# wuji3/visiondk

Measured on AMD Instinct MI355X. Metric: images/sec fwd+bwd+optimizer step (ViT-B/16, bs=256 per GPU), higher is better.
Workload: dtype fp16; 1 GPU; ViT-B/16 ICT, synthetic ImageNet-1k 224x224, random-init weights (reference re-init), per-GPU batch 256, CE label_smoothing 0.05, SGD 0.006/0.937/5e-4, clip 10, EMA on rank 0; global_batch=256, parallelism=dp1

## Files before the change

### visiondk_amd/csrc/norm_loss.hip

```cpp
#include <hip/hip_runtime.h>
#include "vdk_device.h"
#include "vdk_host.h"

__device__ __forceinline__ unsigned ln_q8_pack4(const u32x2 bf, float s, float lim, int fmt, float& am) {
  float c[4];
#pragma unroll
  for (int e = 0; e < 2; ++e) {
    const float a = bf_lo(bf[e]), b = bf_hi(bf[e]);
    am = fmaxf(am, fmaxf(fabsf(a), fabsf(b)));
    c[2 * e] = fminf(fmaxf(a * s, -lim), lim); c[2 * e + 1] = fminf(fmaxf(b * s, -lim), lim);
  }
  int v = 0;
  if (fmt == 0) { v = __builtin_amdgcn_cvt_pk_fp8_f32(c[0], c[1], v, false); v = __builtin_amdgcn_cvt_pk_fp8_f32(c[2], c[3], v, true); }
  else { v = __builtin_amdgcn_cvt_pk_bf8_f32(c[0], c[1], v, false); v = __builtin_amdgcn_cvt_pk_bf8_f32(c[2], c[3], v, true); }
  return (unsigned)v;
}
__device__ __forceinline__ void ln_q8_publish(float am, float* amax, int lane, float* red4) {
#pragma unroll
  for (int off = 1; off < 64; off <<= 1) am = fmaxf(am, __shfl_xor(am, off));
  if (lane == 0) red4[threadIdx.x >> 6] = am;
  __syncthreads();
  if (threadIdx.x == 0 && amax) {
    const float m = fmaxf(fmaxf(red4[0], red4[1]), fmaxf(red4[2], red4[3]));
    if (m > *(volatile float*)amax) atomicMax((unsigned*)amax, __float_as_uint(m));
  }
}
template <bool OUT_BF16 , int MAXJ, bool Q8 = false, int OF = 0>
__global__ __launch_bounds__(256) void ln_fwd_kernel(const float* __restrict__ x, long ldx, int T, int C,
                                                     const float* __restrict__ gamma, const float* __restrict__ beta,
                                                     float eps, void* __restrict__ y, long ldy, float* __restrict__ mean,
                                                     float* __restrict__ rstd, LnQ8 q8 = LnQ8()) {
  const int lane = threadIdx.x & 63;
  __shared__ float q8red[4];
  float q8s = 1.0f, q8lim = 448.0f, q8am = 0.f;
  if (Q8) { q8s = q8.scale ? q8.scale[0] : 1.0f; q8lim = q8.fmt == 0 ? 448.0f : 57344.0f; }
  const int rstride = Q8 ? (int)gridDim.x * 4 : T;
  for (int row = blockIdx.x * 4 + (threadIdx.x >> 6); row < T; row += rstride) {
  const float* xr = x + (long)row * ldx;
  f32x4 v[MAXJ];
#pragma unroll
  for (int j = 0; j < MAXJ; ++j) { const int c = lane * 4 + j * 256; if (c < C) v[j] = *(const f32x4*)(xr + c); }
  float s = 0.f;
#pragma unroll
  for (int j = 0; j < MAXJ; ++j) { const int c = lane * 4 + j * 256; if (c < C) s += (v[j][0] + v[j][1]) + (v[j][2] + v[j][3]); }
  const float mu = wave_sum(s) / (float)C;
  float q = 0.f;
#pragma unroll
  for (int j = 0; j < MAXJ; ++j) {
    const int c = lane * 4 + j * 256;
    if (c < C) {
#pragma unroll
      for (int e = 0; e < 4; ++e) { float d = v[j][e] - mu; q = fmaf(d, d, q); }
    }
  }
  const float rs = 1.0f / sqrtf(wave_sum(q) / (float)C + eps);
  if (lane == 0) { if (mean) mean[row] = mu; if (rstd) rstd[row] = rs; }
#pragma unroll
  for (int j = 0; j < MAXJ; ++j) {
    const int c = lane * 4 + j * 256;
    if (c < C) {
      f32x4 g = *(const f32x4*)(gamma + c), b = *(const f32x4*)(beta + c);
      float o[4];
#pragma unroll
      for (int e = 0; e < 4; ++e) o[e] = (v[j][e] - mu) * rs * g[e] + b[e];
      if (OUT_BF16) {
        const u32x2 ob = {pack_op2<OF>(o[0], o[1]), pack_op2<OF>(o[2], o[3])};
        *(u32x2*)((bf16_t*)y + (long)row * ldy + c) = ob;
        if (Q8) *(unsigned*)(q8.out + (long)row * q8.ld + c) = ln_q8_pack4(ob, q8s, q8lim, q8.fmt, q8am);
      }
      else *(f32x4*)((float*)y + (long)row * ldy + c) = (f32x4){o[0], o[1], o[2], o[3]};
    }
  }
  }
  if (Q8) ln_q8_publish(q8am, q8.amax, lane, q8red);
}

template <bool OUT_BF16, int OF = 0>
__global__ __launch_bounds__(256) void ln_fwd_narrow_kernel(const float* __restrict__ x, long ldx, int T, int C, const float* __restrict__ gamma,
                                                            const float* __restrict__ beta, float eps, void* __restrict__ y, long ldy, float* __restrict__ mean,
                                                            float* __restrict__ rstd) {
  const int row = blockIdx.x * 8 + (threadIdx.x >> 5);
  const int l32 = threadIdx.x & 31, c = l32 * 4;
  const bool on = row < T && c < C;
  f32x4 v = {0.f, 0.f, 0.f, 0.f};
  if (on) v = *(const f32x4*)(x + (long)row * ldx + c);
  float s = on ? (v[0] + v[1]) + (v[2] + v[3]) : 0.f;
#pragma unroll
  for (int o = 16; o >= 1; o >>= 1) s += __shfl_xor(s, o);
  const float mu = s / (float)C;
  float q = 0.f;
  if (on) {
#pragma unroll
    for (int e = 0; e < 4; ++e) { float d = v[e] - mu; q = fmaf(d, d, q); }
  }
#pragma unroll
  for (int o = 16; o >= 1; o >>= 1) q += __shfl_xor(q, o);
  const float rs = 1.0f / sqrtf(q / (float)C + eps);
  if (row < T && l32 == 0) { if (mean) mean[row] = mu; if (rstd) rstd[row] = rs; }
  if (on) {
    f32x4 g = *(const f32x4*)(gamma + c), b = *(const f32x4*)(beta + c);
    float o4[4];
#pragma unroll
    for (int e = 0; e < 4; ++e) o4[e] = (v[e] - mu) * rs * g[e] + b[e];
    if (OUT_BF16) *(u32x2*)((bf16_t*)y + (long)row * ldy + c) = (u32x2){pack_op2<OF>(o4[0], o4[1]), pack_op2<OF>(o4[2], o4[3])};
    else *(f32x4*)((float*)y + (long)row * ldy + c) = (f32x4){o4[0], o4[1], o4[2], o4[3]};
  }
}

template <int MAXJ, bool DY_BF16 , bool OCS, bool Q8 = false, int OF = 0 , int NR = 1,
          bool HALF = false, bool DR16 = false >
__global__ __launch_bounds__(256) void ln_bwd_kernel(const void* __restrict__ dy, long lddy, const float* __restrict__ x,
                                                     long ldx, const float* __restrict__ mean, const float* __restrict__ rstd,
                                                     const float* __restrict__ gamma, const float* __restrict__ dres,
                                                     long lddres, int T, int C, int rows_per_block, float* __restrict__ dx,
                                                     long lddx, bf16_t* __restrict__ dxb, long lddxb,
                                                     float* __restrict__ pgamma, float* __restrict__ pbeta, float* __restrict__ pout, LnQ8 q8 = LnQ8(),
                                                     const float* __restrict__ dy_scale = nullptr ,
                                                     const float* __restrict__ dxb_rs = nullptr , int dxb_rps = 1,
                                                     const bf16_t* __restrict__ dres16 = nullptr) {
  static_assert(!HALF || MAXJ == 1, "HALF: one 128-column slab");
  __shared__ float red[4][MAXJ * 256];
  float q8s = 1.0f, q8lim = 448.0f, q8am = 0.f;
  if (Q8) { q8s = q8.scale ? q8.scale[0] : 1.0f; q8lim = q8.fmt == 0 ? 448.0f : 57344.0f; }
  const int w = threadIdx.x >> 6, lane = threadIdx.x & 63;
  constexpr int HS = HALF ? 2 : 1, RW = NR * HS;
  const int cl = HALF ? (lane & 31) : lane, sub = HALF ? (lane >> 5) : 0;
  const int r0 = blockIdx.x * rows_per_block;
  int r1 = r0 + rows_per_block; if (r1 > T) r1 = T;
  float ag[MAXJ][4], ab[MAXJ][4], ao[OCS ? MAXJ : 1][4];
#pragma unroll
  for (int j = 0; j < MAXJ; ++j)
#pragma unroll
    for (int e = 0; e < 4; ++e) { ag[j][e] = 0.f; ab[j][e] = 0.f; if (OCS) ao[j][e] = 0.f; }
  const float invC = 1.0f / (float)C;
  const float dsc = dy_scale ? dy_scale[0] : 1.0f;
  for (int rb = r0 + w * RW; rb < r1; rb += 4 * RW) {
    float rs[NR], s1[NR], s2[NR];
    float gk[NR][MAXJ][4], xh[NR][MAXJ][4], rv[NR][MAXJ][4];
#pragma unroll
    for (int k = 0; k < NR; ++k) {
      const int row = rb + k * HS + sub;
      const bool ok = row < r1;
      const float mu = ok ? mean[row] : 0.f;
      rs[k] = ok ? rstd[row] : 0.f;
      s1[k] = 0.f; s2[k] = 0.f;
#pragma unroll
      for (int j = 0; j < MAXJ; ++j) {
        const int c = cl * 4 + j * 256;
#pragma unroll
        for (int e = 0; e < 4; ++e) { gk[k][j][e] = 0.f; xh[k][j][e] = 0.f; rv[k][j][e] = 0.f; }
        if (ok && c < C) {
          f32x4 xv = *(const f32x4*)(x + (long)row * ldx + c);
          f32x4 gm = *(const f32x4*)(gamma + c);
          float d[4];
          if (DY_BF16) {
            u32x2 u = *(const u32x2*)((const bf16_t*)dy + (long)row * lddy + c);
            d[0] = op_lo<OF>(u[0]); d[1] = op_hi<OF>(u[0]); d[2] = op_lo<OF>(u[1]); d[3] = op_hi<OF>(u[1]);
          } else {
            f32x4 u = *(const f32x4*)((const float*)dy + (long)row * lddy + c);
            d[0] = u[0]; d[1] = u[1]; d[2] = u[2]; d[3] = u[3];
          }
          if (dy_scale) { d[0] *= dsc; d[1] *= dsc; d[2] *= dsc; d[3] *= dsc; }
          if (DR16) {
            const u32x2 r2 = *(const u32x2*)(dres16 + (long)row * lddres + c);
            rv[k][j][0] = op_lo<OF>(r2[0]); rv[k][j][1] = op_hi<OF>(r2[0]); rv[k][j][2] = op_lo<OF>(r2[1]); rv[k][j][3] = op_hi<OF>(r2[1]);
          } else if (dres) {
            f32x4 r4 = *(const f32x4*)(dres + (long)row * lddres + c);
            rv[k][j][0] = r4[0]; rv[k][j][1] = r4[1]; rv[k][j][2] = r4[2]; rv[k][j][3] = r4[3];
          }
#pragma unroll
          for (int e = 0; e < 4; ++e) {
            float h = (xv[e] - mu) * rs[k];
            float g = d[e] * gm[e];
            xh[k][j][e] = h; gk[k][j][e] = g;
            s1[k] += g; s2[k] = fmaf(g, h, s2[k]);
            ag[j][e] = fmaf(d[e], h, ag[j][e]);
            ab[j][e] += d[e];
          }
        }
      }
    }
#pragma unroll
    for (int k = 0; k < NR; ++k) {
#pragma unroll
      for (int m = HALF ? 16 : 32; m >= 1; m >>= 1) { s1[k] += __shfl_xor(s1[k], m); s2[k] += __shfl_xor(s2[k], m); }
      s1[k] *= invC; s2[k] *= invC;
    }
#pragma unroll
    for (int k = 0; k < NR; ++k) {
      const int row = rb + k * HS + sub;
      const bool ok = row < r1;
#pragma unroll
      for (int j = 0; j < MAXJ; ++j) {
        const int c = cl * 4 + j * 256;
        if (ok && c < C) {
          float o[4];
#pragma unroll
          for (int e = 0; e < 4; ++e) o[e] = rs[k] * (gk[k][j][e] - s1[k] - xh[k][j][e] * s2[k]) + rv[k][j][e];
          if (dx) *(f32x4*)(dx + (long)row * lddx + c) = (f32x4){o[0], o[1], o[2], o[3]};
          if (dxb) {
            if (dxb_rs) { const float f = dxb_rs[row / dxb_rps]; o[0] *= f; o[1] *= f; o[2] *= f; o[3] *= f; }
            const u32x2 ob = {pack_op2<OF>(o[0], o[1]), pack_op2<OF>(o[2], o[3])};
            *(u32x2*)(dxb + (long)row * lddxb + c) = ob;
            if (OCS) { ao[j][0] += op_lo<OF>(ob[0]); ao[j][1] += op_hi<OF>(ob[0]); ao[j][2] += op_lo<OF>(ob[1]); ao[j][3] += op_hi<OF>(ob[1]); }
            if (Q8) *(unsigned*)(q8.out + (long)row * q8.ld + c) = ln_q8_pack4(ob, q8s, q8lim, q8.fmt, q8am);
          }
        }
      }
    }
  }
  if (Q8) ln_q8_publish(q8am, q8.amax, lane, &red[0][0]);
#pragma unroll
  for (int ph = 0; ph < (OCS ? 3 : 2); ++ph) {
    if (ph) __syncthreads();
#pragma unroll
    for (int j = 0; j < MAXJ; ++j)
#pragma unroll
      for (int e = 0; e < 4; ++e) red[w][j * 256 + lane * 4 + e] = ph == 0 ? ag[j][e] : (ph == 1 ? ab[j][e] : ao[OCS ? j : 0][e]);
    __syncthreads();
    for (int c = threadIdx.x; c < C; c += 256) {
      float v = (red[0][c] + red[1][c]) + (red[2][c] + red[3][c]);
      if (HALF) v += (red[0][c + 128] + red[1][c + 128]) + (red[2][c + 128] + red[3][c + 128]);
      if (ph == 0) pgamma[(long)blockIdx.x * 2 * C + c] = v;
      else if (ph == 1) pbeta[(long)blockIdx.x * 2 * C + c] = v;
      else pout[(long)blockIdx.x * C + c] = v;
    }
  }
}

__global__ __launch_bounds__(512) void reduce_rows_f32_kernel(const float* __restrict__ in, long ld, int S, long n,
                                                              float* __restrict__ out, float scale) {
  __shared__ float red[8][64];
  const int cl = threadIdx.x & 63, rg = threadIdx.x >> 6;
  const long c = (long)blockIdx.x * 64 + cl;
  float s0 = 0.f, s1 = 0.f;
  if (c < n) {
    int k = rg;
    for (; k + 8 < S; k += 16) { s0 += in[(long)k * ld + c]; s1 += in[(long)(k + 8) * ld + c]; }
    if (k < S) s0 += in[(long)k * ld + c];
  }
  red[rg][cl] = s0 + s1;
  __syncthreads();
  if (rg == 0 && c < n)
    out[c] = (((red[0][cl] + red[1][cl]) + (red[2][cl] + red[3][cl])) + ((red[4][cl] + red[5][cl]) + (red[6][cl] + red[7][cl]))) * scale;
}

struct ReduceBatch { VdkReduceJob job[8]; int first_block[9]; int n; };
__global__ __launch_bounds__(512) void reduce_rows_batch_kernel(ReduceBatch b) {
  __shared__ float red[8][64];
  int j = 0;
  while (j + 1 < b.n && (int)blockIdx.x >= b.first_block[j + 1]) ++j;
  const VdkReduceJob jb = b.job[j];
  const int cl = threadIdx.x & 63, rg = threadIdx.x >> 6;
  const long c = (long)((int)blockIdx.x - b.first_block[j]) * 64 + cl;
  float s0 = 0.f, s1 = 0.f;
  if (c < jb.n) {
    int k = rg;
    for (; k + 8 < jb.S; k += 16) { s0 += jb.in[(long)k * jb.ld + c]; s1 += jb.in[(long)(k + 8) * jb.ld + c]; }
    if (k < jb.S) s0 += jb.in[(long)k * jb.ld + c];
  }
  red[rg][cl] = s0 + s1;
  __syncthreads();
  if (rg == 0 && c < jb.n)
    jb.out[c] = (((red[0][cl] + red[1][cl]) + (red[2][cl] + red[3][cl])) + ((red[4][cl] + red[5][cl]) + (red[6][cl] + red[7][cl]))) * jb.scale;
}

__global__ __launch_bounds__(512) void reduce_rows_batch_tall_kernel(ReduceBatch b) {
  __shared__ float red[32][17];
  int j = 0;
  while (j + 1 < b.n && (int)blockIdx.x >= b.first_block[j + 1]) ++j;
  const VdkReduceJob jb = b.job[j];
  const int cl = threadIdx.x & 15, rg = threadIdx.x >> 4;
  const long c = (long)((int)blockIdx.x - b.first_block[j]) * 16 + cl;
  float s0 = 0.f, s1 = 0.f, s2 = 0.f, s3 = 0.f;
  if (c < jb.n) {
    int k = rg;
    for (; k + 96 < jb.S; k += 128) {
      s0 += jb.in[(long)k * jb.ld + c]; s1 += jb.in[(long)(k + 32) * jb.ld + c]; s2 += jb.in[(long)(k + 64) * jb.ld + c]; s3 += jb.in[(long)(k + 96) * jb.ld + c];
    }
    for (; k < jb.S; k += 32) s0 += jb.in[(long)k * jb.ld + c];
  }
  red[rg][cl] = (s0 + s1) + (s2 + s3);
  __syncthreads();
  if (rg == 0 && c < jb.n) {
    float t[8];
#pragma unroll
    for (int g = 0; g < 8; ++g) t[g] = (red[4 * g][cl] + red[4 * g + 1][cl]) + (red[4 * g + 2][cl] + red[4 * g + 3][cl]);
    jb.out[c] = (((t[0] + t[1]) + (t[2] + t[3])) + ((t[4] + t[5]) + (t[6] + t[7]))) * jb.scale;
// ... 248 lines not shown
    return vdk_fail(VDK_EINVAL, "vdk_layernorm_fwd: bad argument (C, ldx, ldy % 4 == 0)");
  if (T == 0) return VDK_OK;
  if (C > 4096) return vdk_fail(VDK_EUNSUPPORTED, "vdk_layernorm_fwd: C <= 4096");
  dim3 grid((unsigned)((T + 3) / 4));
#define LNF(BF, MJ) do { if (f16) hipLaunchKernelGGL((ln_fwd_kernel<true, MJ, false, VDK_OPF_F16>), grid, dim3(256), 0, (hipStream_t)stream, x, (long)ldx, (int)T, (int)C, gamma, beta, eps, y, (long)ldy, mean, rstd); \
                          else hipLaunchKernelGGL((ln_fwd_kernel<BF, MJ>), grid, dim3(256), 0, (hipStream_t)stream, x, (long)ldx, (int)T, (int)C, gamma, beta, eps, y, (long)ldy, mean, rstd); } while (0)
  if (y_dtype != VDK_BF16 && y_dtype != VDK_F32 && y_dtype != VDK_F16) return vdk_fail(VDK_EINVAL, "vdk_layernorm_fwd: bad y_dtype");
  const bool bf = y_dtype == VDK_BF16, f16 = y_dtype == VDK_F16;
  if (C <= 128) {
    const dim3 g8((unsigned)((T + 7) / 8));
    if (f16) hipLaunchKernelGGL((ln_fwd_narrow_kernel<true, VDK_OPF_F16>), g8, dim3(256), 0, (hipStream_t)stream, x, (long)ldx, (int)T, (int)C, gamma, beta, eps, y, (long)ldy, mean, rstd);
    else if (bf) hipLaunchKernelGGL((ln_fwd_narrow_kernel<true>), g8, dim3(256), 0, (hipStream_t)stream, x, (long)ldx, (int)T, (int)C, gamma, beta, eps, y, (long)ldy, mean, rstd);
    else hipLaunchKernelGGL((ln_fwd_narrow_kernel<false>), g8, dim3(256), 0, (hipStream_t)stream, x, (long)ldx, (int)T, (int)C, gamma, beta, eps, y, (long)ldy, mean, rstd);
  }
  else if (C <= 256) { if (bf) LNF(true, 1); else LNF(false, 1); }
  else if (C <= 1024) { if (bf) LNF(true, 4); else LNF(false, 4); }
  else { if (bf) LNF(true, 16); else LNF(false, 16); }
#undef LNF
  return vdk_check_launch("vdk_layernorm_fwd");
}

int vdk_layernorm_fwd_q8(const float* x, int64_t ldx, int32_t T, int32_t C, const float* gamma, const float* beta, float eps, void* y, int64_t ldy, float* mean, float* rstd,
                         void* out8, int64_t ldo8, int32_t out_fmt, const float* out_scale, float* out_amax, void* stream) {
  if (!x || !gamma || !beta || !y || !out8 || T < 0 || C <= 0 || (C & 3) || (ldx & 3) || (ldy & 3) || (ldo8 & 3) || (out_fmt != 0 && out_fmt != 1))
    return vdk_fail(VDK_EINVAL, "vdk_layernorm_fwd_q8: bad argument (C, ldx, ldy, ldo8 % 4 == 0)");
  if (C <= 128 || C > 1024) return vdk_fail(VDK_EUNSUPPORTED, "vdk_layernorm_fwd_q8: 128 < C <= 1024");
  if (T == 0) return VDK_OK;
  const LnQ8 q8 = {(unsigned char*)out8, (long)ldo8, out_scale, out_amax, (int)out_fmt};
  unsigned nblk = (unsigned)((T + 3) / 4); if (nblk > 1024) nblk = 1024;
  if (C <= 256)
    hipLaunchKernelGGL((ln_fwd_kernel<true, 1, true>), dim3(nblk), dim3(256), 0, (hipStream_t)stream, x, (long)ldx, (int)T, (int)C, gamma, beta, eps, y, (long)ldy,
                       mean, rstd, q8);
  else
    hipLaunchKernelGGL((ln_fwd_kernel<true, 4, true>), dim3(nblk), dim3(256), 0, (hipStream_t)stream, x, (long)ldx, (int)T, (int)C, gamma, beta, eps, y, (long)ldy,
                       mean, rstd, q8);
  return vdk_check_launch("vdk_layernorm_fwd_q8");
}

int vdk_reduce_rows_f32(const float* in, int64_t ld, int32_t S, int64_t n, float* out, float scale, void* stream) {
  if (!in || !out || S < 0 || n < 0) return vdk_fail(VDK_EINVAL, "vdk_reduce_rows_f32: bad argument");
  if (n == 0) return VDK_OK;
  hipLaunchKernelGGL(reduce_rows_f32_kernel, dim3((unsigned)((n + 63) / 64)), dim3(512), 0, (hipStream_t)stream, in, (long)ld,
                     (int)S, (long)n, out, scale);
  return vdk_check_launch("vdk_reduce_rows_f32");
}

static inline int ln_bwd_blocks(int T, int C) {
  int nb = (T + 15) / 16;
  const int slots = C <= 768 ? 1024 : 768;
  if (nb > slots) nb = slots;
  if (nb < 1) nb = 1;
  const int rpb = (T + nb - 1) / nb;
  nb = (T + rpb - 1) / rpb;
  return nb;
}
int vdk_layernorm_bwd_workspace_bytes(int32_t T, int32_t C, size_t* bytes) {
  if (!bytes || T < 0 || C <= 0) return vdk_fail(VDK_EINVAL, "vdk_layernorm_bwd_workspace_bytes: bad argument");
  *bytes = (size_t)3 * ln_bwd_blocks(T, C) * C * 4;
  return VDK_OK;
}
static int ln_bwd_impl(const void* dy, int64_t lddy, int32_t dy_dtype, const float* x, int64_t ldx, const float* mean,
                       const float* rstd, const float* gamma, const float* dres, int64_t lddres, int32_t T, int32_t C, float* dx,
                       int64_t lddx, void* dxb, int64_t lddxb, float* dgamma, float* dbeta, void* ws, size_t ws_bytes,
                       void* stream_, VdkReduceJob* deferred, float* dxb_colsum = nullptr, VdkReduceJob* deferred2 = nullptr, const LnQ8* q8 = nullptr, int opf = 0,
                       const float* dy_scale = nullptr, const float* dxb_rs = nullptr, int dxb_rps = 1, const void* dres16 = nullptr) {
  hipStream_t stream = (hipStream_t)stream_;
  if (dres16) {
    if (!(dy_dtype == VDK_F16) || !dxb_colsum || C > 1024 || C <= 512 || q8 || dy_scale || dxb_rs) return vdk_fail(VDK_EINVAL, "vdk_layernorm_bwd: dres16 serves the fp16 column-sum form at 512 < C <= 1024");
  }
  if (dy_dtype == VDK_F16) opf = VDK_OPF_F16;
  if (dy_dtype != VDK_BF16 && dy_dtype != VDK_F32 && dy_dtype != VDK_F16) return vdk_fail(VDK_EINVAL, "vdk_layernorm_bwd: bad dy_dtype");
  if (opf && dy_dtype == VDK_BF16) return vdk_fail(VDK_EINVAL, "vdk_layernorm_bwd: bf16 dy with an fp16 output copy");
  if (!dy || !x || !mean || !rstd || !gamma || !dgamma || !dbeta || T <= 0 || C <= 0 || (C & 3) || C > 4096)
    return vdk_fail(VDK_EINVAL, "vdk_layernorm_bwd: bad argument (C % 4 == 0, C <= 4096)");
  const int nb = ln_bwd_blocks(T, C);
  const bool ocs = dxb_colsum != nullptr;
  if (ocs && (!dxb || !deferred2 || C > 1024)) return vdk_fail(VDK_EINVAL, "vdk_layernorm_bwd: the output column sums need dxb, a job slot and C <= 1024");
  size_t need = (size_t)(ocs ? 3 : 2) * nb * C * 4;
  if (!ws || ws_bytes < need) return vdk_fail(VDK_EWORKSPACE, "vdk_layernorm_bwd: workspace too small");
  float* pg = (float*)ws; float* pb = pg + C;
  float* po = pg + (size_t)2 * nb * C;
  const int rpb = (T + nb - 1) / nb;
  const bool bf = dy_dtype != VDK_F32;
#define LNB(MJ, BF, OC, NR, HF) do { if (opf) hipLaunchKernelGGL((ln_bwd_kernel<MJ, BF, OC, false, VDK_OPF_F16, NR, HF>), dim3((unsigned)nb), dim3(256), 0, stream, dy, (long)lddy, x, (long)ldx, \
                                           mean, rstd, gamma, dres, (long)lddres, (int)T, (int)C, rpb, dx, (long)lddx, (bf16_t*)dxb, (long)lddxb, pg, pb, po, LnQ8(), dy_scale, dxb_rs, dxb_rps); \
                             else hipLaunchKernelGGL((ln_bwd_kernel<MJ, BF, OC, false, VDK_OPF_BF16, NR, HF>), dim3((unsigned)nb), dim3(256), 0, stream, dy, (long)lddy, x, (long)ldx, \
                                           mean, rstd, gamma, dres, (long)lddres, (int)T, (int)C, rpb, dx, (long)lddx, (bf16_t*)dxb, (long)lddxb, pg, pb, po, LnQ8(), dy_scale, dxb_rs, dxb_rps); } while (0)
#define LNB2(MJ, NR, HF) do { if (ocs) { if (bf) LNB(MJ, true, true, NR, HF); else LNB(MJ, false, true, NR, HF); } \
                              else { if (bf) LNB(MJ, true, false, NR, HF); else LNB(MJ, false, false, NR, HF); } } while (0)
  if (q8) {
    if (!ocs || !bf || opf || dy_scale || dxb_rs || !q8->out || (q8->ld & 3)) return vdk_fail(VDK_EINVAL, "vdk_layernorm_bwd: the fp8 copy needs bf16 dy, the column-sum form and ld % 4 == 0");
#define LNBQ(MJ) hipLaunchKernelGGL((ln_bwd_kernel<MJ, true, true, true>), dim3((unsigned)nb), dim3(256), 0, stream, dy, (long)lddy, x, (long)ldx, \
                                    mean, rstd, gamma, dres, (long)lddres, (int)T, (int)C, rpb, dx, (long)lddx, (bf16_t*)dxb, (long)lddxb, pg, pb, po, *q8)
    if (C <= 768) LNBQ(3); else LNBQ(4);
#undef LNBQ
  }
  else if (dres16) {
#define LNB16(MJ) hipLaunchKernelGGL((ln_bwd_kernel<MJ, true, true, false, VDK_OPF_F16, 1, false, true>), dim3((unsigned)nb), dim3(256), 0, stream, dy, (long)lddy, x, (long)ldx, mean, rstd, \
                       gamma, (const float*)nullptr, (long)lddres, (int)T, (int)C, rpb, dx, (long)lddx, (bf16_t*)dxb, (long)lddxb, pg, pb, po, LnQ8(), (const float*)nullptr,          \
                       (const float*)nullptr, 1, (const bf16_t*)dres16)
    if (C <= 768) LNB16(3); else LNB16(4);
#undef LNB16
  }
  else if (C <= 128) LNB2(1, 2, true);
  else if (C <= 256) LNB2(1, 2, false);
  else if (C <= 512) LNB2(2, 2, false);
  else if (C <= 768) LNB2(3, 1, false);
  else if (C <= 1024) LNB2(4, 1, false);
  else { if (bf) LNB(16, true, false, 1, false); else LNB(16, false, false, 1, false); }
#undef LNB2
#undef LNB
  if (ocs) *deferred2 = VdkReduceJob{po, (long)C, nb, (long)C, dxb_colsum, 1.0f};
  if (deferred && dbeta == dgamma + C) {
    *deferred = VdkReduceJob{pg, (long)(2 * C), nb, (long)(2 * C), dgamma, 1.0f};
    return vdk_check_launch("vdk_layernorm_bwd");
  }
  if (deferred) deferred->in = nullptr;
  if (dbeta == dgamma + C) {
    hipLaunchKernelGGL(reduce_rows_f32_kernel, dim3((unsigned)((2 * C + 63) / 64)), dim3(512), 0, stream, (const float*)pg, (long)(2 * C), nb,
                       (long)(2 * C), dgamma, 1.0f);
  } else {
    hipLaunchKernelGGL(reduce_rows_f32_kernel, dim3((unsigned)((C + 63) / 64)), dim3(512), 0, stream, (const float*)pg, (long)(2 * C), nb,
                       (long)C, dgamma, 1.0f);
    hipLaunchKernelGGL(reduce_rows_f32_kernel, dim3((unsigned)((C + 63) / 64)), dim3(512), 0, stream, (const float*)pb, (long)(2 * C), nb,
                       (long)C, dbeta, 1.0f);
  }
  return vdk_check_launch("vdk_layernorm_bwd");
}
int vdk_layernorm_bwd(const void* dy, int64_t lddy, int32_t dy_dtype, const float* x, int64_t ldx, const float* mean,
                      const float* rstd, const float* gamma, const float* dres, int64_t lddres, int32_t T, int32_t C, float* dx,
                      int64_t lddx, void* dxb, int64_t lddxb, float* dgamma, float* dbeta, void* ws, size_t ws_bytes,
                      void* stream_) {
  return ln_bwd_impl(dy, lddy, dy_dtype, x, ldx, mean, rstd, gamma, dres, lddres, T, C, dx, lddx, dxb, lddxb, dgamma, dbeta, ws, ws_bytes, stream_, nullptr);
}

static inline int colsum_splits(int T, int N) {
  const int bx = (N / 8 + 31) / 32;
  int target = 1024 / (bx > 0 ? bx : 1); if (target < 128) target = 128;
  int s = (T + 63) / 64; if (s > target) s = target; if (s < 1) s = 1;
  return s;
}
int vdk_colsum_bf16_workspace_bytes(int32_t T, int32_t N, size_t* bytes) {
  if (!bytes || T < 0 || N <= 0) return vdk_fail(VDK_EINVAL, "vdk_colsum_bf16_workspace_bytes: bad argument");
  *bytes = (size_t)colsum_splits(T, N) * N * 4;
  return VDK_OK;
}
int vdk_colsum_bf16(const void* in, int64_t ld, int32_t T, int32_t N, float* out, void* ws, size_t ws_bytes, void* stream_) {
  return vdk_colsum_16(in, ld, T, N, out, ws, ws_bytes, VDK_OPF_BF16, stream_);
}
}
int vdk_colsum_16(const void* in, int64_t ld, int32_t T, int32_t N, float* out, void* ws, size_t ws_bytes, int opf, void* stream_) {
  hipStream_t stream = (hipStream_t)stream_;
  if (!in || !out || T <= 0 || N <= 0 || (N & 7) || (ld & 7)) return vdk_fail(VDK_EINVAL, "vdk_colsum_bf16: bad argument (N, ld % 8 == 0)");
  const int S = colsum_splits(T, N);
  if (!ws || ws_bytes < (size_t)S * N * 4) return vdk_fail(VDK_EWORKSPACE, "vdk_colsum_bf16: workspace too small");
  const int rps = (T + S - 1) / S;
  if (opf) hipLaunchKernelGGL((colsum_bf16_partial_kernel<false, VDK_OPF_F16>), dim3((unsigned)((N / 8 + 31) / 32), (unsigned)S), dim3(256), 0, stream,
                              (const bf16_t*)in, (long)ld, (int)T, (int)N, rps, (float*)ws, LnQ8());
  else
  hipLaunchKernelGGL(colsum_bf16_partial_kernel<false>, dim3((unsigned)((N / 8 + 31) / 32), (unsigned)S), dim3(256), 0, stream,
                     (const bf16_t*)in, (long)ld, (int)T, (int)N, rps, (float*)ws, LnQ8());
  hipLaunchKernelGGL(reduce_rows_f32_kernel, dim3((unsigned)((N + 63) / 64)), dim3(512), 0, stream, (const float*)ws, (long)N, S,
                     (long)N, out, 1.0f);
  return vdk_check_launch("vdk_colsum_bf16");
}
extern "C" {

int vdk_batchnorm1d_fwd(const float* x, int64_t ldx, int32_t B, int32_t F, const float* gamma, const float* beta, float eps, float momentum,
                        int32_t training, float* running_mean, float* running_var, float* y, int64_t ldy, float* save_mean, float* save_invstd,
                        void* stream) {
  if (!x || !gamma || !beta || !y || B <= 0 || F <= 0 || (!training && (!running_mean || !running_var)))
    return vdk_fail(VDK_EINVAL, "vdk_batchnorm1d_fwd: bad argument");
  if (B >= 256)
    hipLaunchKernelGGL(bnrows_fwd_kernel, dim3((unsigned)((F + BNR_COLS - 1) / BNR_COLS)), dim3(512), 0, (hipStream_t)stream, x, (long)ldx, (int)B, (int)F, gamma,
                       beta, eps, momentum, (int)training, running_mean, running_var, y, (long)ldy, save_mean, save_invstd);
  else
    hipLaunchKernelGGL(bn1d_fwd_kernel, dim3((unsigned)((F + 255) / 256)), dim3(256), 0, (hipStream_t)stream, x, (long)ldx, (int)B, (int)F, gamma, beta, eps,
                       momentum, (int)training, running_mean, running_var, y, (long)ldy, save_mean, save_invstd);
  return vdk_check_launch("vdk_batchnorm1d_fwd");
}
int vdk_batchnorm1d_bwd(const float* dy, int64_t lddy, const float* x, int64_t ldx, int32_t B, int32_t F, const float* gamma, const float* save_mean,
                        const float* save_invstd, float* dx, int64_t lddx, float* dgamma, float* dbeta, void* stream) {
  if (!dy || !x || !gamma || !save_mean || !save_invstd || !dx || !dgamma || !dbeta || B <= 0 || F <= 0)
    return vdk_fail(VDK_EINVAL, "vdk_batchnorm1d_bwd: bad argument");
  if (B >= 256)
    hipLaunchKernelGGL(bnrows_bwd_kernel, dim3((unsigned)((F + BNR_COLS - 1) / BNR_COLS)), dim3(512), 0, (hipStream_t)stream, dy, (long)lddy, x, (long)ldx, (int)B,
                       (int)F, gamma, save_mean, save_invstd, dx, (long)lddx, dgamma, dbeta);
  else
    hipLaunchKernelGGL(bn1d_bwd_kernel, dim3((unsigned)((F + 255) / 256)), dim3(256), 0, (hipStream_t)stream, dy, (long)lddy, x, (long)ldx, (int)B, (int)F,
                       gamma, save_mean, save_invstd, dx, (long)lddx, dgamma, dbeta);
  return vdk_check_launch("vdk_batchnorm1d_bwd");
}

int vdk_softmax_ce_amp(const float* logits, int64_t ldl, int32_t B, int32_t C, const int64_t* ya, const int64_t* yb, float lam,
// ... 114 lines not shown
```

Measured before the change: 7850 images/sec.

## Add exact-width LayerNorm backward path with hoisted gamma and batched loads

Result: no change. 7851 images/sec, median of 3 (+0.0%).

```diff
diff --git a/visiondk_amd/csrc/norm_loss.hip b/visiondk_amd/csrc/norm_loss.hip
--- a/visiondk_amd/csrc/norm_loss.hip
+++ b/visiondk_amd/csrc/norm_loss.hip
@@ -1,4 +1,5 @@
 #include <hip/hip_runtime.h>
+#include <type_traits>
 #include "vdk_device.h"
 #include "vdk_host.h"
 
@@ -107,9 +108,21 @@
   }
 }
 
+template <int MAXJ, bool DY_BF16, bool DR16, int NR>
+struct LnBwdRaw {
+  f32x4 x[NR][MAXJ];
+  typedef typename std::conditional<DY_BF16, u32x2, f32x4>::type DyT;
+  typedef typename std::conditional<DR16, u32x2, f32x4>::type DrT;
+  DyT dy[NR][MAXJ];
+  DrT dr[NR][MAXJ];
+  float mu[NR], rs[NR], f[NR];
+};
+template <int OF> __device__ __forceinline__ void ln_unpack4(const u32x2 u, float d[4]) { d[0] = op_lo<OF>(u[0]); d[1] = op_hi<OF>(u[0]); d[2] = op_lo<OF>(u[1]); d[3] = op_hi<OF>(u[1]); }
+template <int OF> __device__ __forceinline__ void ln_unpack4(const f32x4 u, float d[4]) { d[0] = u[0]; d[1] = u[1]; d[2] = u[2]; d[3] = u[3]; }
 template <int MAXJ, bool DY_BF16 , bool OCS, bool Q8 = false, int OF = 0 , int NR = 1,
-          bool HALF = false, bool DR16 = false >
-__global__ __launch_bounds__(256) void ln_bwd_kernel(const void* __restrict__ dy, long lddy, const float* __restrict__ x,
+          bool HALF = false, bool DR16 = false ,
+          bool EXACT = false >
+__global__ __launch_bounds__(256, !EXACT ? 1 : (MAXJ <= 3 ? 4 : 3) ) void ln_bwd_kernel(const void* __restrict__ dy, long lddy, const float* __restrict__ x,
                                                      long ldx, const float* __restrict__ mean, const float* __restrict__ rstd,
                                                      const float* __restrict__ gamma, const float* __restrict__ dres,
                                                      long lddres, int T, int C, int rows_per_block, float* __restrict__ dx,
@@ -122,11 +135,12 @@
   __shared__ float red[4][MAXJ * 256];
   float q8s = 1.0f, q8lim = 448.0f, q8am = 0.f;
   if (Q8) { q8s = q8.scale ? q8.scale[0] : 1.0f; q8lim = q8.fmt == 0 ? 448.0f : 57344.0f; }
-  const int w = threadIdx.x >> 6, lane = threadIdx.x & 63;
+  const int w = EXACT ? __builtin_amdgcn_readfirstlane((int)(threadIdx.x >> 6)) : (int)(threadIdx.x >> 6), lane = threadIdx.x & 63;
   constexpr int HS = HALF ? 2 : 1, RW = NR * HS;
   const int cl = HALF ? (lane & 31) : lane, sub = HALF ? (lane >> 5) : 0;
   const int r0 = blockIdx.x * rows_per_block;
   int r1 = r0 + rows_per_block; if (r1 > T) r1 = T;
+  typedef LnBwdRaw<MAXJ, DY_BF16, DR16, NR> Raw;
   float ag[MAXJ][4], ab[MAXJ][4], ao[OCS ? MAXJ : 1][4];
 #pragma unroll
   for (int j = 0; j < MAXJ; ++j)
@@ -134,76 +148,167 @@
     for (int e = 0; e < 4; ++e) { ag[j][e] = 0.f; ab[j][e] = 0.f; if (OCS) ao[j][e] = 0.f; }
   const float invC = 1.0f / (float)C;
   const float dsc = dy_scale ? dy_scale[0] : 1.0f;
-  for (int rb = r0 + w * RW; rb < r1; rb += 4 * RW) {
-    float rs[NR], s1[NR], s2[NR];
-    float gk[NR][MAXJ][4], xh[NR][MAXJ][4], rv[NR][MAXJ][4];
-#pragma unroll
-    for (int k = 0; k < NR; ++k) {
-      const int row = rb + k * HS + sub;
-      const bool ok = row < r1;
-      const float mu = ok ? mean[row] : 0.f;
-      rs[k] = ok ? rstd[row] : 0.f;
-      s1[k] = 0.f; s2[k] = 0.f;
-#pragma unroll
-      for (int j = 0; j < MAXJ; ++j) {
-        const int c = cl * 4 + j * 256;
-#pragma unroll
-        for (int e = 0; e < 4; ++e) { gk[k][j][e] = 0.f; xh[k][j][e] = 0.f; rv[k][j][e] = 0.f; }
-        if (ok && c < C) {
-          f32x4 xv = *(const f32x4*)(x + (long)row * ldx + c);
-          f32x4 gm = *(const f32x4*)(gamma + c);
-          float d[4];
-          if (DY_BF16) {
-            u32x2 u = *(const u32x2*)((const bf16_t*)dy + (long)row * lddy + c);
-            d[0] = op_lo<OF>(u[0]); d[1] = op_hi<OF>(u[0]); d[2] = op_lo<OF>(u[1]); d[3] = op_hi<OF>(u[1]);
-          } else {
-            f32x4 u = *(const f32x4*)((const float*)dy + (long)row * lddy + c);
-            d[0] = u[0]; d[1] = u[1]; d[2] = u[2]; d[3] = u[3];
-          }
-          if (dy_scale) { d[0] *= dsc; d[1] *= dsc; d[2] *= dsc; d[3] *= dsc; }
-          if (DR16) {
-            const u32x2 r2 = *(const u32x2*)(dres16 + (long)row * lddres + c);
-            rv[k][j][0] = op_lo<OF>(r2[0]); rv[k][j][1] = op_hi<OF>(r2[0]); rv[k][j][2] = op_lo<OF>(r2[1]); rv[k][j][3] = op_hi<OF>(r2[1]);
-          } else if (dres) {
-            f32x4 r4 = *(const f32x4*)(dres + (long)row * lddres + c);
-            rv[k][j][0] = r4[0]; rv[k][j][1] = r4[1]; rv[k][j][2] = r4[2]; rv[k][j][3] = r4[3];
-          }
-#pragma unroll
-          for (int e = 0; e < 4; ++e) {
-            float h = (xv[e] - mu) * rs[k];
-            float g = d[e] * gm[e];
-            xh[k][j][e] = h; gk[k][j][e] = g;
-            s1[k] += g; s2[k] = fmaf(g, h, s2[k]);
-            ag[j][e] = fmaf(d[e], h, ag[j][e]);
-            ab[j][e] += d[e];
+  if constexpr (!EXACT) {
+    for (int rb = r0 + w * RW; rb < r1; rb += 4 * RW) {
+      float rs[NR], s1[NR], s2[NR];
+      float gk[NR][MAXJ][4], xh[NR][MAXJ][4], rv[NR][MAXJ][4];
+#pragma unroll
+      for (int k = 0; k < NR; ++k) {
+        const int row = rb + k * HS + sub;
+        const bool ok = row < r1;
+        const float mu = ok ? mean[row] : 0.f;
+        rs[k] = ok ? rstd[row] : 0.f;
+        s1[k] = 0.f; s2[k] = 0.f;
+#pragma unroll
+        for (int j = 0; j < MAXJ; ++j) {
+          const int c = cl * 4 + j * 256;
+#pragma unroll
+          for (int e = 0; e < 4; ++e) { gk[k][j][e] = 0.f; xh[k][j][e] = 0.f; rv[k][j][e] = 0.f; }
+          if (ok && c < C) {
+            f32x4 xv = *(const f32x4*)(x + (long)row * ldx + c);
+            f32x4 gm = *(const f32x4*)(gamma + c);
+            float d[4];
+            if (DY_BF16) {
+              u32x2 u = *(const u32x2*)((const bf16_t*)dy + (long)row * lddy + c);
+              d[0] = op_lo<OF>(u[0]); d[1] = op_hi<OF>(u[0]); d[2] = op_lo<OF>(u[1]); d[3] = op_hi<OF>(u[1]);
+            } else {
+              f32x4 u = *(const f32x4*)((const float*)dy + (long)row * lddy + c);
+              d[0] = u[0]; d[1] = u[1]; d[2] = u[2]; d[3] = u[3];
+            }
+            if (dy_scale) { d[0] *= dsc; d[1] *= dsc; d[2] *= dsc; d[3] *= dsc; }
+            if (DR16) {
+              const u32x2 r2 = *(const u32x2*)(dres16 + (long)row * lddres + c);
+              rv[k][j][0] = op_lo<OF>(r2[0]); rv[k][j][1] = op_hi<OF>(r2[0]); rv[k][j][2] = op_lo<OF>(r2[1]); rv[k][j][3] = op_hi<OF>(r2[1]);
+            } else if (dres) {
+              f32x4 r4 = *(const f32x4*)(dres + (long)row * lddres + c);
+              rv[k][j][0] = r4[0]; rv[k][j][1] = r4[1]; rv[k][j][2] = r4[2]; rv[k][j][3] = r4[3];
+            }
+#pragma unroll
+            for (int e = 0; e < 4; ++e) {
+              float h = (xv[e] - mu) * rs[k];
+              float g = d[e] * gm[e];
+              xh[k][j][e] = h; gk[k][j][e] = g;
+              s1[k] += g; s2[k] = fmaf(g, h, s2[k]);
+              ag[j][e] = fmaf(d[e], h, ag[j][e]);
+              ab[j][e] += d[e];
+            }
           }
         }
       }
-    }
-#pragma unroll
-    for (int k = 0; k < NR; ++k) {
-#pragma unroll
-      for (int m = HALF ? 16 : 32; m >= 1; m >>= 1) { s1[k] += __shfl_xor(s1[k], m); s2[k] += __shfl_xor(s2[k], m); }
-      s1[k] *= invC; s2[k] *= invC;
-    }
-#pragma unroll
-    for (int k = 0; k < NR; ++k) {
-      const int row = rb + k * HS + sub;
-      const bool ok = row < r1;
-#pragma unroll
-      for (int j = 0; j < MAXJ; ++j) {
-        const int c = cl * 4 + j * 256;
-        if (ok && c < C) {
-          float o[4];
-#pragma unroll
-          for (int e = 0; e < 4; ++e) o[e] = rs[k] * (gk[k][j][e] - s1[k] - xh[k][j][e] * s2[k]) + rv[k][j][e];
-          if (dx) *(f32x4*)(dx + (long)row * lddx + c) = (f32x4){o[0], o[1], o[2], o[3]};
-          if (dxb) {
-            if (dxb_rs) { const float f = dxb_rs[row / dxb_rps]; o[0] *= f; o[1] *= f; o[2] *= f; o[3] *= f; }
-            const u32x2 ob = {pack_op2<OF>(o[0], o[1]), pack_op2<OF>(o[2], o[3])};
-            *(u32x2*)(dxb + (long)row * lddxb + c) = ob;
-            if (OCS) { ao[j][0] += op_lo<OF>(ob[0]); ao[j][1] += op_hi<OF>(ob[0]); ao[j][2] += op_lo<OF>(ob[1]); ao[j][3] += op_hi<OF>(ob[1]); }
-            if (Q8) *(unsigned*)(q8.out + (long)row * q8.ld + c) = ln_q8_pack4(ob, q8s, q8lim, q8.fmt, q8am);
+#pragma unroll
+      for (int k = 0; k < NR; ++k) {
+#pragma unroll
+        for (int m = HALF ? 16 : 32; m >= 1; m >>= 1) { s1[k] += __shfl_xor(s1[k], m); s2[k] += __shfl_xor(s2[k], m); }
+        s1[k] *= invC; s2[k] *= invC;
+      }
+#pragma unroll
+      for (int k = 0; k < NR; ++k) {
+        const int row = rb + k * HS + sub;
+        const bool ok = row < r1;
+#pragma unroll
+        for (int j = 0; j < MAXJ; ++j) {
+          const int c = cl * 4 + j * 256;
+          if (ok && c < C) {
+            float o[4];
+#pragma unroll
+            for (int e = 0; e < 4; ++e) o[e] = rs[k] * (gk[k][j][e] - s1[k] - xh[k][j][e] * s2[k]) + rv[k][j][e];
+            if (dx) *(f32x4*)(dx + (long)row * lddx + c) = (f32x4){o[0], o[1], o[2], o[3]};
+            if (dxb) {
+              if (dxb_rs) { const float f = dxb_rs[row / dxb_rps]; o[0] *= f; o[1] *= f; o[2] *= f; o[3] *= f; }
+              const u32x2 ob = {pack_op2<OF>(o[0], o[1]), pack_op2<OF>(o[2], o[3])};
+              *(u32x2*)(dxb + (long)row * lddxb + c) = ob;
+              if (OCS) { ao[j][0] += op_lo<OF>(ob[0]); ao[j][1] += op_hi<OF>(ob[0]); ao[j][2] += op_lo<OF>(ob[1]); ao[j][3] += op_hi<OF>(ob[1]); }
+              if (Q8) *(unsigned*)(q8.out + (long)row * q8.ld + c) = ln_q8_pack4(ob, q8s, q8lim, q8.fmt, q8am);
+            }
+          }
+        }
+      }
+    }
+  } else {
+    const int c0 = cl * 4;
+    f32x4 gmr[MAXJ];
+#pragma unroll
+    for (int j = 0; j < MAXJ; ++j) {
+      gmr[j] = *(const f32x4*)(gamma + c0 + j * 256);
+    }
+    auto request = [&](int rbv, Raw& R) {
+      const int rb = __builtin_amdgcn_readfirstlane(rbv);
+#pragma unroll
+      for (int k = 0; k < NR; ++k) {
+        int row = rb + k * HS + sub; if (RW > 1 && row >= r1) row = r1 - 1;
+        R.mu[k] = mean[row]; R.rs[k] = rstd[row];
+        R.f[k] = dxb_rs ? dxb_rs[row / dxb_rps] : 1.0f;
+#pragma unroll
+        for (int j = 0; j < MAXJ; ++j) {
+          const int c = c0 + j * 256;
+          R.x[k][j] = *(const f32x4*)(x + (long)row * ldx + c);
+          if (DY_BF16) R.dy[k][j] = *(const typename Raw::DyT*)((const bf16_t*)dy + (long)row * lddy + c);
+          else R.dy[k][j] = *(const typename Raw::DyT*)((const float*)dy + (long)row * lddy + c);
+          if (DR16) R.dr[k][j] = *(const typename Raw::DrT*)(dres16 + (long)row * lddres + c);
+          else if (dres) R.dr[k][j] = *(const typename Raw::DrT*)(dres + (long)row * lddres + c);
+          else R.dr[k][j] = 0;
+        }
+      }
+    };
+    Raw cur;
+    for (int rb = r0 + w * RW; rb < r1; rb += 4 * RW) {
+      request(rb, cur);
+      float s1[NR], s2[NR], xh[NR][MAXJ][4];
+#pragma unroll
+      for (int k = 0; k < NR; ++k) {
+        const bool ok = RW == 1 || rb + k * HS + sub < r1;
+        const float mu = cur.mu[k], rs = cur.rs[k];
+        s1[k] = 0.f; s2[k] = 0.f;
+#pragma unroll
+        for (int j = 0; j < MAXJ; ++j) {
+          const f32x4 gm = gmr[j];
+          float d[4];
+          ln_unpack4<OF>(cur.dy[k][j], d);
+          if (dy_scale) { d[0] *= dsc; d[1] *= dsc; d[2] *= dsc; d[3] *= dsc; }
+#pragma unroll
+          for (int e = 0; e < 4; ++e) {
+            const float h = ok ? (cur.x[k][j][e] - mu) * rs : 0.f;
+            const float de = ok ? d[e] : 0.f;
+            const float g = de * gm[e];
+            xh[k][j][e] = h;
+            s1[k] += g; s2[k] = fmaf(g, h, s2[k]);
+            ag[j][e] = fmaf(de, h, ag[j][e]);
+            ab[j][e] += de;
+          }
+        }
+      }
+      __builtin_amdgcn_sched_barrier(0);
+#pragma unroll
+      for (int k = 0; k < NR; ++k) {
+#pragma unroll
+        for (int m = HALF ? 16 : 32; m >= 1; m >>= 1) { s1[k] += __shfl_xor(s1[k], m); s2[k] += __shfl_xor(s2[k], m); }
+        s1[k] *= invC; s2[k] *= invC;
+      }
+      __builtin_amdgcn_sched_barrier(0);
+#pragma unroll
+      for (int k = 0; k < NR; ++k) {
+        const int row = rb + k * HS + sub;
+        const bool ok = RW == 1 || row < r1;
+        const float rs = cur.rs[k];
+#pragma unroll
+        for (int j = 0; j < MAXJ; ++j) {
+          const int c = c0 + j * 256;
+          if (ok) {
+            const f32x4 gm = gmr[j];
+            float d[4], rv[4], o[4];
+            ln_unpack4<OF>(cur.dy[k][j], d);
+            if (dy_scale) { d[0] *= dsc; d[1] *= dsc; d[2] *= dsc; d[3] *= dsc; }
+            ln_unpack4<OF>(cur.dr[k][j], rv);
+#pragma unroll
+            for (int e = 0; e < 4; ++e) { const float g = d[e] * gm[e]; o[e] = rs * (g - s1[k] - xh[k][j][e] * s2[k]) + rv[e]; }
+            if (dx) *(f32x4*)(dx + (long)row * lddx + c) = (f32x4){o[0], o[1], o[2], o[3]};
+            if (dxb) {
+              if (dxb_rs) { const float f = cur.f[k]; o[0] *= f; o[1] *= f; o[2] *= f; o[3] *= f; }
+              const u32x2 ob = {pack_op2<OF>(o[0], o[1]), pack_op2<OF>(o[2], o[3])};
+              *(u32x2*)(dxb + (long)row * lddxb + c) = ob;
+              if (OCS) { ao[j][0] += op_lo<OF>(ob[0]); ao[j][1] += op_hi<OF>(ob[0]); ao[j][2] += op_lo<OF>(ob[1]); ao[j][3] += op_hi<OF>(ob[1]); }
+              if (Q8) *(unsigned*)(q8.out + (long)row * q8.ld + c) = ln_q8_pack4(ob, q8s, q8lim, q8.fmt, q8am);
+            }
           }
         }
       }
@@ -618,25 +723,32 @@
   float* po = pg + (size_t)2 * nb * C;
   const int rpb = (T + nb - 1) / nb;
   const bool bf = dy_dtype != VDK_F32;
-#define LNB(MJ, BF, OC, NR, HF) do { if (opf) hipLaunchKernelGGL((ln_bwd_kernel<MJ, BF, OC, false, VDK_OPF_F16, NR, HF>), dim3((unsigned)nb), dim3(256), 0, stream, dy, (long)lddy, x, (long)ldx, \
+#define LNBX(MJ, BF, OC, NR, HF, EX) do { if (opf) hipLaunchKernelGGL((ln_bwd_kernel<MJ, BF, OC, false, VDK_OPF_F16, NR, HF, false, EX>), dim3((unsigned)nb), dim3(256), 0, stream, dy, (long)lddy, x, (long)ldx, \
                                            mean, rstd, gamma, dres, (long)lddres, (int)T, (int)C, rpb, dx, (long)lddx, (bf16_t*)dxb, (long)lddxb, pg, pb, po, LnQ8(), dy_scale, dxb_rs, dxb_rps); \
-                             else hipLaunchKernelGGL((ln_bwd_kernel<MJ, BF, OC, false, VDK_OPF_BF16, NR, HF>), dim3((unsigned)nb), dim3(256), 0, stream, dy, (long)lddy, x, (long)ldx, \
+                             else hipLaunchKernelGGL((ln_bwd_kernel<MJ, BF, OC, false, VDK_OPF_BF16, NR, HF, false, EX>), dim3((unsigned)nb), dim3(256), 0, stream, dy, (long)lddy, x, (long)ldx, \
                                            mean, rstd, gamma, dres, (long)lddres, (int)T, (int)C, rpb, dx, (long)lddx, (bf16_t*)dxb, (long)lddxb, pg, pb, po, LnQ8(), dy_scale, dxb_rs, dxb_rps); } while (0)
+#define LNB(MJ, BF, OC, NR, HF) do { if (MJ <= 4 && C == ((HF) ? 128 : MJ * 256)) LNBX(MJ, BF, OC, NR, HF, (MJ <= 4)); else LNBX(MJ, BF, OC, NR, HF, false); } while (0)
 #define LNB2(MJ, NR, HF) do { if (ocs) { if (bf) LNB(MJ, true, true, NR, HF); else LNB(MJ, false, true, NR, HF); } \
                               else { if (bf) LNB(MJ, true, false, NR, HF); else LNB(MJ, false, false, NR, HF); } } while (0)
   if (q8) {
     if (!ocs || !bf || opf || dy_scale || dxb_rs || !q8->out || (q8->ld & 3)) return vdk_fail(VDK_EINVAL, "vdk_layernorm_bwd: the fp8 copy needs bf16 dy, the column-sum form and ld % 4 == 0");
-#define LNBQ(MJ) hipLaunchKernelGGL((ln_bwd_kernel<MJ, true, true, true>), dim3((unsigned)nb), dim3(256), 0, stream, dy, (long)lddy, x, (long)ldx, \
+#define LNBQ(MJ) LNBQX(MJ, C == MJ * 256)
+#define LNBQX(MJ, EX) if (EX) LNBQ1(MJ, true); else LNBQ1(MJ, false)
+#define LNBQ1(MJ, EX) hipLaunchKernelGGL((ln_bwd_kernel<MJ, true, true, true, VDK_OPF_BF16, 1, false, false, EX>), dim3((unsigned)nb), dim3(256), 0, stream, dy, (long)lddy, x, (long)ldx, \
                                     mean, rstd, gamma, dres, (long)lddres, (int)T, (int)C, rpb, dx, (long)lddx, (bf16_t*)dxb, (long)lddxb, pg, pb, po, *q8)
     if (C <= 768) LNBQ(3); else LNBQ(4);
 #undef LNBQ
+#undef LNBQX
+#undef LNBQ1
   }
   else if (dres16) {
-#define LNB16(MJ) hipLaunchKernelGGL((ln_bwd_kernel<MJ, true, true, false, VDK_OPF_F16, 1, false, true>), dim3((unsigned)nb), dim3(256), 0, stream, dy, (long)lddy, x, (long)ldx, mean, rstd, \
+#define LNB16(MJ) do { if (C == MJ * 256) LNB16X(MJ, true); else LNB16X(MJ, false); } while (0)
+#define LNB16X(MJ, EX) hipLaunchKernelGGL((ln_bwd_kernel<MJ, true, true, false, VDK_OPF_F16, 1, false, true, EX>), dim3((unsigned)nb), dim3(256), 0, stream, dy, (long)lddy, x, (long)ldx, mean, rstd, \
                        gamma, (const float*)nullptr, (long)lddres, (int)T, (int)C, rpb, dx, (long)lddx, (bf16_t*)dxb, (long)lddxb, pg, pb, po, LnQ8(), (const float*)nullptr,          \
                        (const float*)nullptr, 1, (const bf16_t*)dres16)
     if (C <= 768) LNB16(3); else LNB16(4);
 #undef LNB16
+#undef LNB16X
   }
   else if (C <= 128) LNB2(1, 2, true);
   else if (C <= 256) LNB2(1, 2, false);
@@ -646,6 +758,7 @@
   else { if (bf) LNB(16, true, false, 1, false); else LNB(16, false, false, 1, false); }
 #undef LNB2
 #undef LNB
+#undef LNBX
   if (ocs) *deferred2 = VdkReduceJob{po, (long)C, nb, (long)C, dxb_colsum, 1.0f};
   if (deferred && dbeta == dgamma + C) {
     *deferred = VdkReduceJob{pg, (long)(2 * C), nb, (long)(2 * C), dgamma, 1.0f};
```
